# HyTruongSon/GraphFlow

Hardware: AMD Instinct MI355X
Metric: CCN-2D (SMP_omega) molecules/sec fwd+bwd (higher is better)
Workload: dtype f32 (level block products: 2xf16-split operands, 22-bit, fp32 accumulate); 1 GPU; cfg3: SMP_omega 3 levels, C=64, F=5, D=5, cap=29, batch=1024 synthetic QM9-size molecules/GPU, device-resident, fused levels; parallelism=single GPU

## Files before the change

### graphflow_amd/csrc/gf_internal.h

```cpp
#ifndef GF_INTERNAL_H_INCLUDED
#define GF_INTERNAL_H_INCLUDED

#include <hip/hip_runtime.h>

#include <cstdarg>
#include <cstddef>
#include <cstdio>
#include <cstdlib>
#include <unordered_map>
#include <vector>

#include "gf_hip.h"

struct gf_dist_state;

struct gf_ctx {
    int device = 0;
    gf_dist_state *dist = nullptr;
    int fp32_products = 0;
    int r18_generic = 0;
    hipStream_t stream = nullptr;
    bool owns_stream = false;
    void *ws = nullptr;
    size_t ws_bytes = 0;
    void *stage = nullptr;
    size_t stage_bytes = 0;
    void *repack = nullptr;
    size_t repack_bytes = 0;
    void *pinned = nullptr;
    size_t pinned_bytes = 0;
    char err[512] = {0};
    bool timing = false;
    char timing_filter[64] = {0};
    struct Timer {
        const char *name;
        double ms;
        long long launches;
    };
    struct Pending {
        int slot;
        hipEvent_t start, stop;
    };
    std::vector<Timer> timers;
    std::vector<Pending> pending;
    std::vector<hipEvent_t> event_pool;
};

namespace gf {

gf_status fail(gf_ctx *ctx, gf_status st, const char *fmt, ...);
inline bool env_is(const char *name, char v) {
    const char *e = std::getenv(name);
    return e && e[0] == v;
}
bool poison_buffers();
gf_status ensure_ws(gf_ctx *ctx, size_t bytes);
gf_status ensure_stage(gf_ctx *ctx, size_t bytes);
gf_status ensure_repack(gf_ctx *ctx, size_t bytes);
gf_status ensure_pinned(gf_ctx *ctx, size_t bytes);
gf_status opt_in_lds_fn(gf_ctx *ctx, const void *kernel, size_t bytes);
template <typename Kern>
gf_status opt_in_lds(gf_ctx *ctx, Kern kern, size_t bytes) {
    return opt_in_lds_fn(ctx, reinterpret_cast<const void *>(kern), bytes);
}
bool dist_active(const gf_ctx *ctx);
bool dist_poisoned(const gf_ctx *ctx);
gf_status dist_allreduce_on(gf_ctx *ctx, float *buf, size_t n, hipStream_t stream, const char *what = nullptr);
gf_status dist_wait_event(gf_ctx *ctx, hipEvent_t ev, const char *where);
hipStream_t dist_stream(gf_ctx *ctx);

#ifndef GF_NT_SITES
#define GF_NT_SITES 124
#endif
#if defined(__HIPCC__)
template <int SITE, typename V>
__device__ __forceinline__ V gf_ld_s(const V *p) {
    if constexpr ((GF_NT_SITES & SITE) != 0) return __builtin_nontemporal_load(p);
    else return *p;
}
template <int SITE, typename V>
__device__ __forceinline__ void gf_st_s(V *p, V v) {
    if constexpr ((GF_NT_SITES & SITE) != 0) __builtin_nontemporal_store(v, p);
    else *p = v;
}
#endif

#define GF_HIP_TRY(ctx, expr)                                                                      \
    do {                                                                                           \
        hipError_t e__ = (expr);                                                                   \
        if (e__ != hipSuccess)                                                                     \
            return gf::fail((ctx), GF_ERR_HIP, "%s failed: %s (%s:%d)", #expr, hipGetErrorString(e__), \
                            __FILE__, __LINE__);                                                   \
    } while (0)

#define GF_LAUNCH_CHECK(ctx, what)                                                                  \
    do {                                                                                            \
        hipError_t e__ = hipGetLastError();                                                         \
        if (e__ != hipSuccess)                                                                      \
            return gf::fail((ctx), GF_ERR_HIP, "launch of %s failed: %s", (what), hipGetErrorString(e__)); \
    } while (0)

struct LaunchTimer {
    gf_ctx *ctx;
    int slot = -1;
    hipEvent_t start = nullptr, stop = nullptr;
    hipStream_t stream = nullptr;
    LaunchTimer(gf_ctx *c, const char *name, hipStream_t on = nullptr);
    void done();
};
gf_status resolve_timers(gf_ctx *ctx);

#define GF_LAUNCH(ctx, name, kern, grid, block, lds, ...)                                  \
    do {                                                                                   \
        gf::LaunchTimer lt__((ctx), (name));                                               \
        hipLaunchKernelGGL(kern, grid, block, lds, (ctx)->stream, __VA_ARGS__);           \
        lt__.done();                                                                       \
        GF_LAUNCH_CHECK((ctx), (name));                                                    \
    } while (0)

static inline size_t align_up(size_t x, size_t a) { return (x + a - 1) / a * a; }

gf_status r18_forward(gf_ctx *ctx, const float *P, const float *A, float *Out, int N, int C, int batch);
gf_status r18_backward(gf_ctx *ctx, const float *G, const float *A, float *dP, int N, int C, int batch, int accumulate);
size_t r18_workspace_bytes(int N, int C, int batch);
struct gf_ragged_nodes {
    const int *pair_node;
    const int *node_s;
    const long long *node_p, *node_row, *node_pair;
    long long total_rows, total_pairs;
};
bool r18_ragged_supported(int smax, int C, const void *p0, const void *p1);
size_t r18_ragged_workspace_bytes(long long total_rows, long long total_pairs, int C);
gf_status r18_forward_ragged(gf_ctx *ctx, const float *P, const float *A, float *Out, const gf_ragged_nodes &t,
                             long long pair_lo, long long pair_hi, int smax, int C);
gf_status r18_backward_ragged(gf_ctx *ctx, const float *G, const float *A, float *dP, const gf_ragged_nodes &t,
                              long long pair_lo, long long pair_hi, int smax, int C, int accumulate);
gf_status family_forward(gf_ctx *ctx, int K, const float *P, const float *A, float *Out, int N, int C, int batch);
gf_status family_backward(gf_ctx *ctx, int K, const float *G, const float *A, float *dP, int N, int C, int batch,
                          int accumulate);
size_t family_workspace_bytes(int K, int N, int C, int batch);

}
#endif
```

### graphflow_amd/csrc/smp_level_c64_split.hip

```cpp
#include <cstdlib>
#include <type_traits>

#include "gemm_lds.h"
#include "gf_internal.h"
#include "smp_internal.h"

namespace gf {
namespace {

using lds_image::f16v;
using lds_image::f4v;
typedef _Float16 h8 __attribute__((ext_vector_type(8)));
typedef _Float16 h2 __attribute__((ext_vector_type(2)));
typedef float f2v __attribute__((ext_vector_type(2)));

constexpr int kSpThreads = 512;

template <unsigned EMIN = 14u>
__device__ __forceinline__ void pow2_scale(unsigned maxbits, float *s, float *inv) {
    unsigned e = maxbits >> 23;
    e = e < EMIN ? EMIN : e;
    *s = __uint_as_float((267u - e) << 23);
    *inv = __uint_as_float((e - 13u) << 23);
}
// ... 85 lines not shown
        else
            build_weight_images<false, 1, 16>(w, H, L, winv, wmax, threadIdx.x);
    } else {
        if (blockIdx.x == 0)
            build_weight_images<true, 1, 32>(w, H, L, winv, wmax, threadIdx.x);
        else
            build_weight_images<false, 1, 32>(w, H, L, winv, wmax, threadIdx.x);
    }
}

__global__ __launch_bounds__(kSpThreads) void smp_split_weight_images_c128(SplitImages a) {
    __shared__ unsigned wmax[1];
    const int q = blockIdx.z >> 3, pos = blockIdx.z & 7, i = q >> 1, j = q & 1;
    uint4 *out = a.img[blockIdx.y] + (size_t)(2 * q + blockIdx.x) * kSpImgStride128;
    float *winv = reinterpret_cast<float *>(out + 2 * kSpAll128) + pos;
    const float *w = a.Wst[blockIdx.y] + (size_t)pos * 128 * 128;
    uint4 *H = out + pos * 512, *L = out + kSpAll128 + pos * 512;
    if (blockIdx.x == 0)
        build_weight_images<true, 1, 64, 128>(w + (size_t)64 * i * 128 + 64 * j, H, L, winv, wmax, threadIdx.x);
    else
        build_weight_images<false, 1, 64, 128>(w + (size_t)64 * j * 128 + 64 * i, H, L, winv, wmax, threadIdx.x);
}

#ifndef GF_SP_WHOLE_PANEL
#define GF_SP_WHOLE_PANEL 16
#endif
template <bool FWD, bool MASK, int CB = 64, int NF = 2, int NX = 0, bool CLS = false, int W = 1, bool ACC = false>
__global__ __launch_bounds__(kSpThreads, 1) void smp_rowpanel_split(const float *__restrict__ A, const float *__restrict__ rs,
                                                                     const float *__restrict__ Wst, float *__restrict__ Out, int rows,
                                                                     const int *__restrict__ trow, int store_mask,
                                                                     const uint4 *__restrict__ wimg,
                                                                     const int *__restrict__ rcls,
                                                                     int a_off, int out_off) {
    static_assert(W == 1 || (CB == 64 && NF == 2 && NX == 0 && !CLS), "sub-block passes: 64-channel panels, plain row factors");
    static_assert(W > 1 || !ACC, "");
    static_assert(!CLS || (!FWD && MASK && CB == 64 && NF == 2 && NX == 0), "row classes: the masked backward products at 64 channels");
    constexpr int LDA = (FWD ? 4 * CB : 2 * CB) * W, LDOUT = (FWD ? 2 * CB : 4 * CB) * W, BS = CB * W;
    if constexpr (W == 1) a_off = out_off = 0;
    constexpr int ALL = W == 1 ? kSpAll : kSpAll128;
    constexpr int VPL = CB / 2, NC = CB / 16, NH = CB >= 32 ? CB / 32 : 1, E = NH * NC * 64;
    auto t_row = [](int t) { return MASK ? (t & 0x1fffffff) : t; };
    auto t_own = [](int t) { return MASK ? t < 0 : true; };
    auto t_tr = [](int t) { return MASK ? ((t >> 30) & 1) != 0 : true; };
    auto t_bc = [](int t) { return MASK ? ((t >> 29) & 1) != 0 : true; };
    static_assert(NX == 0 || (NX == 3 && CB <= 32 && NF == 2), "the extra products: prebuilt images, plain row factors");
    constexpr int NP = 8 + NX;
    extern __shared__ __attribute__((aligned(16))) uint4 sp_smem[];
    uint4 *imgH = sp_smem, *imgL = sp_smem + NP * E;
    float *winv = reinterpret_cast<float *>(sp_smem + 2 * NP * E);
    unsigned *wmax = reinterpret_cast<unsigned *>(winv + 16);
    float *facs = winv + 32;
    const int tid = threadIdx.x, lane = tid & 63, li = lane & 31, lh = lane >> 5;
    const int wave = tid >> 6;
    typedef unsigned long long u64x2 __attribute__((ext_vector_type(2)));
    unsigned long long *rowp = reinterpret_cast<unsigned long long *>(facs + (kSpThreads / 64) * 32);

    if (wimg) {
        for (int t = tid; t < NP * E; t += kSpThreads) {
            const int pos = t / E, g = (pos < 8 ? pos : kSpStacked + pos - 8) * 512 + t % E;
            imgH[t] = wimg[g];
            imgL[t] = wimg[ALL + g];
        }
        if (tid < 2) reinterpret_cast<uint4 *>(winv)[tid] = wimg[2 * ALL + tid];
        if (NX > 0 && tid < NX) winv[8 + tid] = reinterpret_cast<const float *>(wimg + 2 * kSpAll)[kSpStacked + tid];
    } else {
        static_assert(E == 512 || true, "");
        if constexpr (CB == 64) build_weight_images<FWD, 8>(Wst, imgH, imgL, winv, wmax, tid);
    }
    __syncthreads();

    const int npanels = (rows + 31) / 32;
    const int nwaves = gridDim.x * (kSpThreads / 64);
    float *myfac = facs + wave * 32;

    struct Raw {
        f4v a[VPL / 4];
    };
    struct Spl {
        uint4 h[NC], l[NC];
    };
    auto load_raw_at = [&](Raw &R, int src_row, int blk, bool present) {
        __builtin_amdgcn_sched_barrier(0);
        asm volatile("" : "+v"(src_row));
        const float *src = A + (size_t)src_row * LDA + blk * BS + a_off + VPL * lh;
        if constexpr (MASK) src = present ? src : sp_zero_page;
#pragma unroll
        for (int q = 0; q < VPL / 4; ++q) R.a[q] = gf_ld_s<1>(reinterpret_cast<const f4v *>(src + 4 * q));
        __builtin_amdgcn_sched_barrier(0);
    };
    auto load_raw = [&](Raw &R, int p, int blk, bool present) {
        const int row = p * 32 + li;
        load_raw_at(R, row < rows ? row : rows - 1, blk, present);
    };
    auto fetch_trow = [&](int p) {
        const int row = p * 32 + li;
        return trow[row < rows ? row : rows - 1];
    };
    struct RowFac {
        float f[8];
    };
    auto load_scale = [&](int p) {
        int row = p * 32 + li;
        row = row < rows ? row : rows - 1;
        RowFac r;
        if constexpr (NF == 8) {
            const f4v a = *reinterpret_cast<const f4v *>(rs + (size_t)row * 8), b = *reinterpret_cast<const f4v *>(rs + (size_t)row * 8 + 4);
            r.f[0] = a[0], r.f[1] = a[1], r.f[2] = a[2], r.f[3] = a[3], r.f[4] = b[0], r.f[5] = b[1], r.f[6] = b[2], r.f[7] = b[3];
        } else {
            const float2 t = *reinterpret_cast<const float2 *>(rs + (size_t)row * 2);
            r.f[0] = r.f[1] = t.x, r.f[2] = t.y;
            r.f[3] = r.f[4] = r.f[5] = r.f[6] = r.f[7] = 1.f;
        }
        return r;
    };
    auto split_blk = [&](const Raw &R, Spl &S, float &inv) {
        __builtin_amdgcn_sched_barrier(0);
        unsigned m = 0u;
#pragma unroll
        for (int q = 0; q < VPL / 4; ++q)
#pragma unroll
            for (int j = 0; j < 4; ++j) {
                const unsigned b = __float_as_uint(R.a[q][j]) & 0x7fffffffu;
                m = b > m ? b : m;
            }
        const unsigned mo = (unsigned)__shfl_xor((int)m, 32);
        m = mo > m ? mo : m;
        float s;
        pow2_scale(m, &s, &inv);
#pragma unroll
        for (int c = 0; c < NC; ++c) {
            unsigned hw[4], lw[4];
#pragma unroll
            for (int j = 0; j < 4; ++j) {
                h2 h, l;
                const f4v v = R.a[2 * c + (j >> 1)];
                split_pair(v[2 * (j & 1)], v[2 * (j & 1) + 1], s, &h, &l);
                hw[j] = __builtin_bit_cast(unsigned, h);
                lw[j] = __builtin_bit_cast(unsigned, l);
            }
            S.h[c] = make_uint4(hw[0], hw[1], hw[2], hw[3]);
            S.l[c] = make_uint4(lw[0], lw[1], lw[2], lw[3]);
        }
        __builtin_amdgcn_sched_barrier(0);
    };
    auto prod = [&](const Spl &S, float rowfac, int wpos, f16v &acc0, f16v &acc1) {
        __builtin_amdgcn_wave_barrier();
        myfac[li] = rowfac * winv[wpos];
        __builtin_amdgcn_wave_barrier();
        const uint4 *bh = imgH + (size_t)wpos * E + lane, *bl = imgL + (size_t)wpos * E + lane;
#pragma unroll
        for (int nh = 0; nh < NH; ++nh) {
            f16v t;
#pragma unroll
            for (int r = 0; r < 16; ++r) t[r] = 0.f;
#pragma unroll
            for (int c = 0; c < NC; ++c) {
                const h8 bhc = __builtin_bit_cast(h8, bh[(NC * nh + c) * 64]), blc = __builtin_bit_cast(h8, bl[(NC * nh + c) * 64]);
                const h8 ah = __builtin_bit_cast(h8, S.h[c]), al = __builtin_bit_cast(h8, S.l[c]);
                t = __builtin_amdgcn_mfma_f32_32x32x16_f16(al, bhc, t, 0, 0, 0);
                t = __builtin_amdgcn_mfma_f32_32x32x16_f16(ah, blc, t, 0, 0, 0);
            }
#pragma unroll
            for (int r = 0; r < 16; ++r) t[r] *= kLowUnscale;
#pragma unroll
            for (int c = 0; c < NC; ++c) {
                const h8 bhc = __builtin_bit_cast(h8, bh[(NC * nh + c) * 64]);
                const h8 ah = __builtin_bit_cast(h8, S.h[c]);
                t = __builtin_amdgcn_mfma_f32_32x32x16_f16(ah, bhc, t, 0, 0, 0);
            }
            f16v &acc = nh ? acc1 : acc0;
#pragma unroll
            for (int g = 0; g < 4; ++g) {
                const f4v fac = *reinterpret_cast<const f4v *>(myfac + 8 * g + 4 * lh);
#pragma unroll
                for (int j = 0; j < 4; ++j) acc[4 * g + j] += t[4 * g + j] * fac[j];
            }
        }
        __builtin_amdgcn_wave_barrier();
    };
    auto clear = [&](f16v &acc0, f16v &acc1) {
#pragma unroll
        for (int r = 0; r < 16; ++r) acc0[r] = acc1[r] = 0.f;
    };
    auto start = [&](int p, int o, f16v &acc0, f16v &acc1, auto full) {
        if constexpr (!ACC) {
            clear(acc0, acc1);
        } else {
            const int r0 = p * 32;
            const float *out = Out + (size_t)(r0 + 4 * lh) * LDOUT + o * BS + out_off + li;
#pragma unroll
            for (int r = 0; r < 16; ++r) {
                const int rr = (r & 3) + 8 * (r >> 2);
                const bool ok = decltype(full)::value || r0 + 4 * lh + rr < rows;
                acc0[r] = ok ? out[(size_t)rr * LDOUT] : 0.f;
                acc1[r] = ok ? out[(size_t)rr * LDOUT + 32] : 0.f;
            }
        }
    };
    auto store_out = [&](int p, int o, const f16v &acc0, const f16v &acc1, auto full, unsigned rowbits = 0xffffffffu) {
        const int r0 = p * 32;
        float *out = Out + (size_t)(r0 + 4 * lh) * LDOUT + o * BS + out_off + li;
        if constexpr (CB < 32)
            out = li < CB ? out : sp_dump + (size_t)((r0 & 255) + 4 * lh) * 64 + li;
        if constexpr (MASK && !FWD && decltype(full)::value) {
            if (rowbits != 0xffffffffu) {
                const unsigned mine = rowbits >> (4 * lh);
                float *dump = sp_dump + (size_t)((r0 & 255) + 4 * lh) * 64 + li;
#pragma unroll
                for (int r = 0; r < 16; ++r) {
                    const int rr = (r & 3) + 8 * (r >> 2);
                    float *dst = ((mine >> rr) & 1u) ? out + (size_t)rr * LDOUT : dump + rr * 64;
                    gf_st_s<2>(dst, acc0[r]);
                    if constexpr (NH == 2) gf_st_s<2>(dst + 32, acc1[r]);
                }
                return;
            }
        }
        if constexpr (decltype(full)::value) {
#pragma unroll
            for (int r = 0; r < 16; ++r) {
                const int rr = (r & 3) + 8 * (r >> 2);
                gf_st_s<2>(out + (size_t)rr * LDOUT, acc0[r]);
                if constexpr (NH == 2) gf_st_s<2>(out + (size_t)rr * LDOUT + 32, acc1[r]);
            }
        } else {
            const unsigned mine = (MASK && !FWD) ? rowbits >> (4 * lh) : 0xffffffffu;
#pragma unroll
            for (int r = 0; r < 16; ++r) {
                const int rr = (r & 3) + 8 * (r >> 2);
                if (r0 + 4 * lh + rr < rows && li < CB && ((mine >> rr) & 1u)) {
                    gf_st_s<2>(out + (size_t)rr * LDOUT, acc0[r]);
                    if constexpr (NH == 2) gf_st_s<2>(out + (size_t)rr * LDOUT + 32, acc1[r]);
                }
            }
        }
    };

    int tnext = CLS ? 0 : fetch_trow(blockIdx.x * (kSpThreads / 64) + wave);
    auto panel = [&](int p, Raw &Ra, Raw &Rb, auto full) {
        const int pn = p + nwaves;
        const int tcur = tnext;
        tnext = fetch_trow(pn);
        const RowFac sc = load_scale(p);
        f16v acc0, acc1;
        Spl X, Y, Z;
        float iX, iY, iZ;
        if (FWD) {
            split_blk(Ra, X, iX);
            load_raw(Ra, p, 1, t_bc(tcur));
            split_blk(Rb, Z, iZ);
            load_raw(Rb, p, 2, t_own(tcur));
            start(p, 1, acc0, acc1, full);
            prod(X, iX * sc.f[5], 5, acc0, acc1);
            prod(Z, iZ * sc.f[7], 7, acc0, acc1);
            split_blk(Ra, Y, iY);
            prod(Y, iY * sc.f[6], 6, acc0, acc1);
            store_out(p, 1, acc0, acc1, full);
            start(p, 0, acc0, acc1, full);
            prod(X, iX * sc.f[0], 0, acc0, acc1);
            prod(X, iX * sc.f[2], 2, acc0, acc1);
            prod(Y, iY * sc.f[1], 1, acc0, acc1);
            if constexpr (NX == 3) {
                prod(X, iX, 8, acc0, acc1);
                prod(Y, iY, 9, acc0, acc1);
                prod(Y, iY * sc.f[2], 10, acc0, acc1);
            }
            load_raw(Ra, p, 3, t_bc(tcur));
            split_blk(Rb, Z, iZ);
            load_raw_at(Rb, t_row(tnext), 0, t_tr(tnext));
            prod(Z, iZ * sc.f[3], 3, acc0, acc1);
            split_blk(Ra, Z, iZ);
            load_raw(Ra, pn, 0, t_own(tnext));
            prod(Z, iZ * sc.f[4], 4, acc0, acc1);
            store_out(p, 0, acc0, acc1, full);
        } else {
            split_blk(Ra, X, iX);
            split_blk(Rb, Y, iY);
            const unsigned rowbits = (MASK && store_mask) ? (unsigned)__ballot(t_own(tcur)) : 0xffffffffu;
            start(p, 2, acc0, acc1, full);
            prod(X, iX * sc.f[3], 3, acc0, acc1);
            store_out(p, 2, acc0, acc1, full, rowbits);
            start(p, 3, acc0, acc1, full);
            prod(X, iX * sc.f[4], 4, acc0, acc1);
            store_out(p, 3, acc0, acc1, full);
            start(p, 1, acc0, acc1, full);
            prod(X, iX * sc.f[1], 1, acc0, acc1);
            prod(Y, iY * sc.f[6], 6, acc0, acc1);
            if constexpr (NX == 3) {
                prod(X, iX, 9, acc0, acc1);
                prod(X, iX * sc.f[2], 10, acc0, acc1);
            }
            store_out(p, 1, acc0, acc1, full);
            load_raw_at(Ra, t_row(tcur), 1, !(MASK && store_mask) || t_own(tcur));
            load_raw(Rb, pn, 1, !(MASK && store_mask) || t_bc(tnext));
            start(p, 0, acc0, acc1, full);
            prod(X, iX * sc.f[0], 0, acc0, acc1);
            prod(X, iX * sc.f[2], 2, acc0, acc1);
            prod(Y, iY * sc.f[5], 5, acc0, acc1);
            if constexpr (NX == 3) prod(X, iX, 8, acc0, acc1);
            split_blk(Ra, Z, iZ);
            load_raw(Ra, pn, 0, !(MASK && store_mask) || t_bc(tnext));
            prod(Z, iZ * sc.f[7], 7, acc0, acc1);
            store_out(p, 0, acc0, acc1, full, rowbits);
        }
    };
    if constexpr (CLS) {
        const int n_own_p = (rcls[0] + 31) >> 5, n_tot_p = n_own_p + ((rcls[1] + 31) >> 5), n_ent = 32 * n_tot_p;
        const int2 *ent = reinterpret_cast<const int2 *>(rcls + 4);
        unsigned long long *myrow = rowp + wave * 32;
        auto fetch_entry = [&](int q, int *rw) {
            const int i = q * 32 + li;
            const int2 e = ent[i < n_ent ? i : n_ent - 1];
            *rw = e.x;
            return e.y;
        };
        auto e_row = [](int rw) { return rw & 0x1fffffff; };
        auto scale_at = [&](int row) {
            const float2 t = *reinterpret_cast<const float2 *>(rs + (size_t)row * 2);
            RowFac r;
            r.f[0] = r.f[1] = t.x, r.f[2] = t.y;
            r.f[3] = r.f[4] = r.f[5] = r.f[6] = r.f[7] = 1.f;
            return r;
        };
        auto post_rows = [&](int rw) {
            __builtin_amdgcn_wave_barrier();
            myrow[li] = reinterpret_cast<unsigned long long>(rw < 0 ? sp_dump + li * 64 : Out + (size_t)e_row(rw) * LDOUT);
            __builtin_amdgcn_wave_barrier();
        };
        auto store_rows = [&](int o, const f16v &acc0, const f16v &acc1) {
#pragma unroll
            for (int g = 0; g < 4; ++g) {
                const u64x2 a = *reinterpret_cast<const u64x2 *>(myrow + 8 * g + 4 * lh), b = *reinterpret_cast<const u64x2 *>(myrow + 8 * g + 4 * lh + 2);
#pragma unroll
                for (int j = 0; j < 4; ++j) {
                    float *dst = reinterpret_cast<float *>(j < 2 ? a[j & 1] : b[j & 1]) + o * CB + li;
                    gf_st_s<2>(dst, acc0[4 * g + j]);
                    gf_st_s<2>(dst + 32, acc1[4 * g + j]);
                }
            }
        };
        int p = blockIdx.x * (kSpThreads / 64) + wave;
        int rnext, tn = fetch_entry(p, &rnext);
        Raw Ra, Rb;
        load_raw_at(Rb, e_row(rnext), 1, t_bc(tn));
        load_raw_at(Ra, e_row(rnext), 0, t_bc(tn));
        auto panel_own = [&](int q) {
            const int qn = q + nwaves, rcur = rnext, tcur = tn;
            tn = fetch_entry(qn, &rnext);
            const RowFac sc = scale_at(e_row(rcur));
            post_rows(rcur);
            f16v acc0, acc1;
            Spl X, Y, Z;
            float iX, iY, iZ;
            split_blk(Ra, X, iX);
            split_blk(Rb, Y, iY);
            clear(acc0, acc1);
            prod(X, iX * sc.f[3], 3, acc0, acc1);
            store_rows(2, acc0, acc1);
            clear(acc0, acc1);
            prod(X, iX * sc.f[4], 4, acc0, acc1);
            store_rows(3, acc0, acc1);
            clear(acc0, acc1);
            prod(X, iX * sc.f[1], 1, acc0, acc1);
            prod(Y, iY * sc.f[6], 6, acc0, acc1);
            store_rows(1, acc0, acc1);
            load_raw_at(Ra, t_row(tcur), 1, t_own(tcur));
            load_raw_at(Rb, e_row(rnext), 1, t_bc(tn));
            clear(acc0, acc1);
            prod(X, iX * sc.f[0], 0, acc0, acc1);
            prod(X, iX * sc.f[2], 2, acc0, acc1);
            prod(Y, iY * sc.f[5], 5, acc0, acc1);
            split_blk(Ra, Z, iZ);
            load_raw_at(Ra, e_row(rnext), 0, t_bc(tn));
            prod(Z, iZ * sc.f[7], 7, acc0, acc1);
            store_rows(0, acc0, acc1);
        };
        auto panel_absent = [&](int q) {
            const int qn = q + nwaves, rcur = rnext;
            tn = fetch_entry(qn, &rnext);
            const RowFac sc = scale_at(e_row(rcur));
            post_rows(rcur);
            f16v acc0, acc1;
            Spl X, Y;
            float iX, iY;
            split_blk(Ra, X, iX);
            split_blk(Rb, Y, iY);
            load_raw_at(Rb, e_row(rnext), 1, t_bc(tn));
            load_raw_at(Ra, e_row(rnext), 0, t_bc(tn));
            clear(acc0, acc1);
            prod(X, iX * sc.f[4], 4, acc0, acc1);
            store_rows(3, acc0, acc1);
            clear(acc0, acc1);
            prod(X, iX * sc.f[1], 1, acc0, acc1);
            prod(Y, iY * sc.f[6], 6, acc0, acc1);
            store_rows(1, acc0, acc1);
        };
        for (; p < n_own_p; p += nwaves) panel_own(p);
        for (; p < n_tot_p; p += nwaves) panel_absent(p);
        return;
    }
    if constexpr (CB <= GF_SP_WHOLE_PANEL) {
        constexpr int NB = FWD ? 5 : 3;
        Raw R[NB];
        int p = blockIdx.x * (kSpThreads / 64) + wave;
        int t1 = tnext, t2 = fetch_trow(p + nwaves);
        auto request = [&](int q, int t) {
            if constexpr (FWD) {
                load_raw(R[0], q, 0, t_own(t));
                load_raw_at(R[1], t_row(t), 0, t_tr(t));
                load_raw(R[2], q, 1, t_bc(t));
                load_raw(R[3], q, 2, t_own(t));
                load_raw(R[4], q, 3, t_bc(t));
            } else {
                const bool all = !(MASK && store_mask);
                load_raw(R[0], q, 0, all || t_bc(t));
                load_raw(R[1], q, 1, all || t_bc(t));
                load_raw_at(R[2], t_row(t), 1, all || t_own(t));
            }
        };
        auto panel16 = [&](int q, auto full) {
// ... 154 lines not shown
                const h8 ah = __builtin_bit_cast(h8, S.h[c]);
                t = __builtin_amdgcn_mfma_f32_32x32x16_f16(ah, bhc, t, 0, 0, 0);
            }
            f16v &acc = nh ? acc1 : acc0;
#pragma unroll
            for (int g = 0; g < 4; ++g) {
                const f4v fac = *reinterpret_cast<const f4v *>(myfac + 8 * g + 4 * lh);
#pragma unroll
                for (int j = 0; j < 4; ++j) acc[4 * g + j] += t[4 * g + j] * fac[j];
            }
        }
        __builtin_amdgcn_wave_barrier();
    };
    const int npanels = (rows + 31) / 32;
    for (int p = wg * (kSmThreads / 64) + wave; p < npanels; p += nwg * (kSmThreads / 64)) {
        const int r0 = p * 32;
        const int row = r0 + li < rows ? r0 + li : rows - 1;
        Raw R[NIN];
#pragma unroll
        for (int k = 0; k < NIN; ++k) {
            const float *src = In + (size_t)row * LDA + k * CB + VPL * lh;
#pragma unroll
            for (int q = 0; q < VPL / 4; ++q) R[k].a[q] = *reinterpret_cast<const f4v *>(src + 4 * q);
        }
        (void)NIN;
        auto store_out = [&](int o, const f16v &acc0, const f16v &acc1) {
            float *out = Out + (size_t)(r0 + 4 * lh) * LDOUT + o * CB + li;
#pragma unroll
            for (int r = 0; r < 16; ++r) {
                const int rr = (r & 3) + 8 * (r >> 2);
                if (r0 + 4 * lh + rr < rows && li < CB) {
                    out[(size_t)rr * LDOUT] = acc0[r];
                    if constexpr (NH == 2) out[(size_t)rr * LDOUT + 32] = acc1[r];
                }
            }
        };
        f16v acc0, acc1;
        Spl X;
        float iX;
        if constexpr (PROG == 0) {
#pragma unroll
            for (int r = 0; r < 16; ++r) acc0[r] = acc1[r] = 0.f;
#pragma unroll
            for (int k = 0; k < NPOS; ++k) {
                split_blk(R[k], X, iX);
                prod(X, iX, k, acc0, acc1);
            }
            store_out(0, acc0, acc1);
        } else if constexpr (PROG == 1) {
            split_blk(R[0], X, iX);
#pragma unroll
            for (int k = 0; k < NPOS; ++k) {
#pragma unroll
                for (int r = 0; r < 16; ++r) acc0[r] = acc1[r] = 0.f;
                prod(X, iX, k, acc0, acc1);
                store_out(k, acc0, acc1);
            }
        } else {
#pragma unroll
            for (int k = 0; k < NPOS; ++k) {
                split_blk(R[k], X, iX);
#pragma unroll
                for (int r = 0; r < 16; ++r) acc0[r] = acc1[r] = 0.f;
                prod(X, iX, k, acc0, acc1);
                store_out(k, acc0, acc1);
            }
        }
    }
}

template <int CB>
__global__ __launch_bounds__(kSmThreads, 2) void smp_small_split(SmallJobs jobs, const uint4 *__restrict__ wimg) {
    int j = 0;
    if (jobs.n > 1 && (int)blockIdx.x >= jobs.wg0[1]) j = 1;
    if (jobs.n > 2 && (int)blockIdx.x >= jobs.wg0[2]) j = 2;
    const int wg = (int)blockIdx.x - jobs.wg0[j];
    switch (jobs.prog[j]) {
        case 0: small_split_body<0, CB>(jobs.In[j], jobs.Out[j], jobs.rows[j], wimg, jobs.pos0[j], wg, jobs.nwg[j]); break;
        case 1: small_split_body<1, CB>(jobs.In[j], jobs.Out[j], jobs.rows[j], wimg, jobs.pos0[j], wg, jobs.nwg[j]); break;
        default: small_split_body<2, CB>(jobs.In[j], jobs.Out[j], jobs.rows[j], wimg, jobs.pos0[j], wg, jobs.nwg[j]); break;
    }
}

constexpr int kWsThreads = 512, kWsSlice = 16, kWsRowWords = 12;
constexpr int kWsACols = 256, kWsBCols = 320;
constexpr int kWsStageWords = 2 * (kWsACols + kWsBCols) * kWsRowWords;
constexpr size_t kWsLds = 2 * (size_t)kWsStageWords * 4 + 2 * (kWsACols + kWsBCols) * sizeof(float);
__constant__ int c_ws_ablk[8] = {0, 1, 0, 2, 3, 0, 1, 0};
__constant__ int c_ws_bblk[8] = {1, 1, 2, 0, 0, 3, 3, 4};

template <int W = 1>
__global__ __launch_bounds__(kWsThreads, 1) void smp_wgrad_split(const float *__restrict__ T, const float *__restrict__ dO,
                                                                  const float *__restrict__ rs, int rows, int kchunk,
                                                                  float *__restrict__ part, const int *__restrict__ trow,
                                                                  const unsigned *__restrict__ cmax,
                                                                  const unsigned *__restrict__ chan,
                                                                  float smax, float max_tot, float max_tr,
                                                                  const unsigned *__restrict__ row_max,
                                                                  int packed,
                                                                  int a_off, int b_off, int out_off) {
    if constexpr (W == 1) a_off = b_off = out_off = 0;
    constexpr int LDT = 256 * W, LDO = 128 * W, BS = 64 * W, LDW = 64 * W;
    extern __shared__ __attribute__((aligned(16))) unsigned ws_smem[];
    const int tid = threadIdx.x, lane = tid & 63, li = lane & 31, lg = lane >> 5;
    const int wave = __builtin_amdgcn_readfirstlane(tid >> 6);
    const int kend = rows;
    auto K = [&](int n) { return (long long)(blockIdx.x + (long long)n * gridDim.x) * kWsSlice; };

    float *sScale = reinterpret_cast<float *>(ws_smem + 2 * kWsStageWords), *sInv = sScale + kWsACols + kWsBCols;
    if (cmax) {
        for (int c = tid; c < kWsACols + kWsBCols; c += kWsThreads) pow2_scale_col(cmax[c], &sScale[c], &sInv[c]);
    } else {
        if (row_max) {
            max_tot = __uint_as_float(row_max[0]);
            max_tr = __uint_as_float(row_max[1]);
        }
        for (int c = tid; c < kWsACols + kWsBCols; c += kWsThreads) {
            const bool isa = c < kWsACols;
            const int blk = (isa ? c : c - kWsACols) >> 6, ch = c & 63;
            const float m = __uint_as_float(chan[(isa ? 0 : 64) + ch]);
            const float fa = blk < 2 ? smax : max_tot;
            const float fb = blk == 0 ? 1.f : blk == 2 ? max_tr : max_tot;
            pow2_scale_col(__float_as_uint(m * (isa ? fa : fb)), &sScale[c], &sInv[c]);
        }
    }
    __syncthreads();

    const int q_lo = lane & 7, pair = lane >> 3;
    struct Task {
        f4v v0, v1;
    };
    constexpr int NB = 2;
    struct Set {
        Task ta, tb[NB];
        float f0[NB], f1[NB];
    };
    const bool has_b1 = wave < 2;
    const int zbit = ((wave >> 1) & 1) == 0 ? 31 : 29;
    const int a_quad = 8 * wave + q_lo;
    auto b_blk = [&](int e) { return (wave + 8 * e) >> 1; };
    auto b_quad = [&](int e) { return 8 * ((wave + 8 * e) & 1) + q_lo; };
    const int rot = (q_lo >> 1) & 3;
    f4v a_scale, b_scale[NB];
#pragma unroll
    for (int i = 0; i < 4; ++i) {
        a_scale[i] = sScale[4 * a_quad + ((i + rot) & 3)];
#pragma unroll
        for (int e = 0; e < NB; ++e) {
            const int blk = b_blk(e) < 5 ? b_blk(e) : 0;
            b_scale[e][i] = sScale[kWsACols + 64 * blk + 4 * b_quad(e) + ((i + rot) & 3)];
        }
    }
    int ia0 = 0, ia1 = 0, ib0 = 0, ib1 = 0;
    auto fetch_trow = [&](int m, int &t0, int &t1) {
        const long long k = K(m) + 2 * pair, last = kend - 1;
        t0 = trow[k < last ? k : last];
        t1 = trow[k + 1 < last ? k + 1 : last];
    };
    auto load_slice = [&](Set &S, int m) {
        const int g0 = packed ? (ia0 & 0x1fffffff) : ia0, g1 = packed ? (ia1 & 0x1fffffff) : ia1;
        const bool z0 = packed && !((ia0 >> zbit) & 1), z1 = packed && !((ia1 >> zbit) & 1);
        const bool zg0 = packed && ia0 >= 0, zg1 = packed && ia1 >= 0;
        ia0 = ib0, ia1 = ib1;
        fetch_trow(m + 2, ib0, ib1);
        const long long last = kend - 1, kk = K(m) + 2 * pair;
        const int c0 = (int)(kk < last ? kk : last), c1 = (int)(kk + 1 < last ? kk + 1 : last);
        const int a_col = W == 1 ? 4 * a_quad : (a_quad >> 4) * BS + a_off + ((4 * a_quad) & 63);
        const float *t0 = T + (size_t)c0 * LDT + a_col, *t1 = T + (size_t)c1 * LDT + a_col;
        S.ta.v0 = gf_ld_s<4>(reinterpret_cast<const f4v *>(z0 ? sp_zero_page + 4 * q_lo : t0));
        S.ta.v1 = gf_ld_s<4>(reinterpret_cast<const f4v *>(z1 ? sp_zero_page + 4 * q_lo : t1));
#pragma unroll
        for (int e = 0; e < NB; ++e) {
            const int blk = b_blk(e);
            S.f0[e] = rs[(size_t)c0 * 2 + (blk == 2)];
            S.f1[e] = rs[(size_t)c1 * 2 + (blk == 2)];
            const bool gathered = blk == 4;
            const float *src = blk < 5 ? dO + (blk >= 3 ? BS : 0) + b_off + 4 * b_quad(e) : T + a_col;
            const int ld = blk < 5 ? LDO : LDT;
            const float *s0 = src + (size_t)(gathered ? g0 : c0) * ld, *s1 = src + (size_t)(gathered ? g1 : c1) * ld;
            S.tb[e].v0 = gf_ld_s<256>(reinterpret_cast<const f4v *>((gathered && zg0) ? sp_zero_page + 4 * q_lo : s0));
            S.tb[e].v1 = gf_ld_s<256>(reinterpret_cast<const f4v *>((gathered && zg1) ? sp_zero_page + 4 * q_lo : s1));
        }
    };
    auto rotate = [&](f4v v) {
        if (rot & 1) v = f4v{v[1], v[2], v[3], v[0]};
        if (rot & 2) v = f4v{v[2], v[3], v[0], v[1]};
        return v;
    };
    auto store_task = [&](const f4v &v0, const f4v &v1, unsigned *H, unsigned *L, int col0, const f4v &sc, float f0, float f1) {
        const f4v r0 = rotate(v0), r1 = rotate(v1);
#pragma unroll
        for (int i = 0; i < 4; ++i) {
            h2 h, l;
            split_plain2(r0[i], r1[i], sc[i] * f0, sc[i] * f1, &h, &l);
            const int w = (col0 + ((i + rot) & 3)) * kWsRowWords + pair;
            H[w] = __builtin_bit_cast(unsigned, h);
            L[w] = __builtin_bit_cast(unsigned, l);
        }
    };
    auto store_slice = [&](const Set &S, long long k0, unsigned *stage) {
        unsigned *Ah = stage, *Al = Ah + kWsACols * kWsRowWords, *Bh = Al + kWsACols * kWsRowWords, *Bl = Bh + kWsBCols * kWsRowWords;
        const long long k = k0 + 2 * pair;
        const float ok0 = k < kend ? 1.f : 0.f, ok1 = k + 1 < kend ? 1.f : 0.f;
        store_task(S.ta.v0, S.ta.v1, Ah, Al, 4 * a_quad, a_scale, ok0, ok1);
#pragma unroll
        for (int e = 0; e < NB; ++e) {
            if (e == 1 && !has_b1) break;
            const int blk = b_blk(e);
            const bool scaled = blk == 1 || blk == 2;
            const float m0 = scaled ? S.f0[e] : 1.f, m1 = scaled ? S.f1[e] : 1.f;
            store_task(S.tb[e].v0, S.tb[e].v1, Bh, Bl, 64 * blk + 4 * b_quad(e), b_scale[e], ok0 * m0, ok1 * m1);
        }
    };

    f16v acc[2][2];
#pragma unroll
    for (int r = 0; r < 16; ++r) acc[0][0][r] = acc[0][1][r] = acc[1][0][r] = acc[1][1][r] = 0.f;
    const int ablk = c_ws_ablk[wave], bblk = c_ws_bblk[wave];
    auto products = [&](const unsigned *stage) {
        const unsigned *Ah = stage, *Al = Ah + kWsACols * kWsRowWords, *Bh = Al + kWsACols * kWsRowWords, *Bl = Bh + kWsBCols * kWsRowWords;
        const int ao = (ablk * 64 + li) * kWsRowWords + 4 * lg, bo = (bblk * 64 + li) * kWsRowWords + 4 * lg;
        h8 ah[2], al[2], bh[2], bl[2];
#pragma unroll
        for (int t = 0; t < 2; ++t) {
            ah[t] = __builtin_bit_cast(h8, *reinterpret_cast<const uint4 *>(Ah + ao + t * 32 * kWsRowWords));
            al[t] = __builtin_bit_cast(h8, *reinterpret_cast<const uint4 *>(Al + ao + t * 32 * kWsRowWords));
            bh[t] = __builtin_bit_cast(h8, *reinterpret_cast<const uint4 *>(Bh + bo + t * 32 * kWsRowWords));
            bl[t] = __builtin_bit_cast(h8, *reinterpret_cast<const uint4 *>(Bl + bo + t * 32 * kWsRowWords));
        }
#pragma unroll
        for (int mt = 0; mt < 2; ++mt)
#pragma unroll
            for (int nt = 0; nt < 2; ++nt) {
                acc[mt][nt] = __builtin_amdgcn_mfma_f32_32x32x16_f16(al[mt], bh[nt], acc[mt][nt], 0, 0, 0);
                acc[mt][nt] = __builtin_amdgcn_mfma_f32_32x32x16_f16(ah[mt], bl[nt], acc[mt][nt], 0, 0, 0);
                acc[mt][nt] = __builtin_amdgcn_mfma_f32_32x32x16_f16(ah[mt], bh[nt], acc[mt][nt], 0, 0, 0);
            }
    };
    auto interval = [&](Set &Ra, int n) {
        store_slice(Ra, K(n + 1), ws_smem + ((n + 1) & 1) * kWsStageWords);
        load_slice(Ra, n + 4);
        products(ws_smem + (n & 1) * kWsStageWords);
        __syncthreads();
    };
    if (K(0) < kend) {
        Set S0, S1, S2;
        fetch_trow(0, ia0, ia1);
        fetch_trow(1, ib0, ib1);
        load_slice(S0, 0);
        load_slice(S1, 1);
        load_slice(S2, 2);
        store_slice(S0, K(0), ws_smem);
        load_slice(S0, 3);
        __syncthreads();
        int left = (int)((kend - K(0) + (long long)gridDim.x * kWsSlice - 1) / ((long long)gridDim.x * kWsSlice));
        int n = 0;
        for (; left >= 3; n += 3, left -= 3) {
            interval(S1, n);
            interval(S2, n + 1);
            interval(S0, n + 2);
        }
        if (left >= 1) interval(S1, n);
        if (left >= 2) interval(S2, n + 1);
    }
    float *out = part + ((size_t)blockIdx.x * 8 + wave) * (LDW * LDW) + out_off + li;
    const float *ia = sInv + ablk * 64, *ib = sInv + kWsACols + bblk * 64;
#pragma unroll
    for (int mt = 0; mt < 2; ++mt)
#pragma unroll
        for (int nt = 0; nt < 2; ++nt) {
            const float ub = ib[32 * nt + li];
#pragma unroll
            for (int r = 0; r < 16; ++r) {
                const int row = 32 * mt + (r & 3) + 8 * (r >> 2) + 4 * lg;
                out[row * LDW + 32 * nt] = acc[mt][nt][r] * (ia[row] * ub);
            }
        }
}


constexpr long long kTrowWindow = (long long)kFusedMaxField * kFusedMaxField;
constexpr int kW8Threads = 256;
template <int CB, int NF, int NX = 0>
__global__ __launch_bounds__(kW8Threads, 1) void smp_wgrad_all(const float *__restrict__ T, const float *__restrict__ dO,
                                                                const float *__restrict__ rs, int rows, float *__restrict__ part,
                                                                const int *__restrict__ trow, const unsigned *__restrict__ cmax,
                                                                const unsigned *__restrict__ chan, float smax,
                                                                const unsigned *__restrict__ row_max, int packed, float *__restrict__ xpart = nullptr) {
    static_assert(CB == 32 || CB == 16, "one 32 x 32 tile per product");
    static_assert(NX == 0 || (NX == 3 && NF == 2), "the extra products take the plain (tot, tr) row factors");
    constexpr int NP = 8 + NX;
    constexpr int ACOLS = 4 * CB, BCOLS = 5 * CB;
    constexpr int SL = CB == 16 ? 2 * kWsSlice : kWsSlice;
    constexpr int TROW = 16 * CB, DROW = 8 * CB;
    constexpr int NBF = NF == 8 ? 8 : 5;
    __shared__ float sScale[ACOLS + BCOLS], sInv[ACOLS + BCOLS];
    __shared__ float sImg[NP * CB * CB];
    const int tid = threadIdx.x, lane = tid & 63, li = lane & 31, lg = lane >> 5;
    const int wave = __builtin_amdgcn_readfirstlane(tid >> 6);
    const int hi = (CB == 16 && li >= 16) ? 1 : 0;
    const int lc = CB == 16 ? (li & 15) : li;
    const int rb = 8 * lg + 16 * hi;
    if (cmax) {
        for (int c = tid; c < ACOLS + BCOLS; c += kW8Threads) pow2_scale_col(cmax[c], &sScale[c], &sInv[c]);
    } else {
        const float max_tot = __uint_as_float(row_max[0]), max_tr = __uint_as_float(row_max[1]);
        for (int c = tid; c < ACOLS + BCOLS; c += kW8Threads) {
            const bool isa = c < ACOLS;
            const int blk = (isa ? c : c - ACOLS) / CB, ch = c % CB;
            const float m = __uint_as_float(chan[(isa ? 0 : CB) + ch]);
            const float fa = blk < 2 ? smax : max_tot;
// ... 577 lines not shown
```

Baseline: 155,700 molecules/s.

## Swizzle weight-gradient LDS staging layout and tag global pointers with address space

```diff
diff --git a/graphflow_amd/csrc/gf_internal.h b/graphflow_amd/csrc/gf_internal.h
--- a/graphflow_amd/csrc/gf_internal.h
+++ b/graphflow_amd/csrc/gf_internal.h
@@ -83,6 +83,25 @@
     if constexpr ((GF_NT_SITES & SITE) != 0) __builtin_nontemporal_store(v, p);
     else *p = v;
 }
+#define GF_GLOBAL __attribute__((address_space(1)))
+template <typename V>
+__device__ __forceinline__ const GF_GLOBAL V *gf_global(const V *p) {
+    return (const GF_GLOBAL V *)p;
+}
+template <typename V>
+__device__ __forceinline__ GF_GLOBAL V *gf_global(V *p) {
+    return (GF_GLOBAL V *)p;
+}
+template <int SITE, typename V>
+__device__ __forceinline__ V gf_ld_g(const GF_GLOBAL V *p) {
+    if constexpr ((GF_NT_SITES & SITE) != 0) return __builtin_nontemporal_load(p);
+    else return *p;
+}
+template <int SITE, typename V>
+__device__ __forceinline__ void gf_st_g(GF_GLOBAL V *p, V v) {
+    if constexpr ((GF_NT_SITES & SITE) != 0) __builtin_nontemporal_store(v, p);
+    else *p = v;
+}
 #endif
 
 #define GF_HIP_TRY(ctx, expr)                                                                      \
diff --git a/graphflow_amd/csrc/smp_level_c64_split.hip b/graphflow_amd/csrc/smp_level_c64_split.hip
--- a/graphflow_amd/csrc/smp_level_c64_split.hip
+++ b/graphflow_amd/csrc/smp_level_c64_split.hip
@@ -191,10 +191,11 @@
     auto load_raw_at = [&](Raw &R, int src_row, int blk, bool present) {
         __builtin_amdgcn_sched_barrier(0);
         asm volatile("" : "+v"(src_row));
-        const float *src = A + (size_t)src_row * LDA + blk * BS + a_off + VPL * lh;
-        if constexpr (MASK) src = present ? src : sp_zero_page;
-#pragma unroll
-        for (int q = 0; q < VPL / 4; ++q) R.a[q] = gf_ld_s<1>(reinterpret_cast<const f4v *>(src + 4 * q));
+        unsigned long long sa = (unsigned long long)(A + (size_t)src_row * LDA + blk * BS + a_off + VPL * lh);
+        if constexpr (MASK) sa = present ? sa : (unsigned long long)sp_zero_page;
+        const GF_GLOBAL float *src = (const GF_GLOBAL float *)sa;
+#pragma unroll
+        for (int q = 0; q < VPL / 4; ++q) R.a[q] = gf_ld_g<1>(reinterpret_cast<const GF_GLOBAL f4v *>(src + 4 * q));
         __builtin_amdgcn_sched_barrier(0);
     };
     auto load_raw = [&](Raw &R, int p, int blk, bool present) {
@@ -282,7 +283,10 @@
             for (int g = 0; g < 4; ++g) {
                 const f4v fac = *reinterpret_cast<const f4v *>(myfac + 8 * g + 4 * lh);
 #pragma unroll
-                for (int j = 0; j < 4; ++j) acc[4 * g + j] += t[4 * g + j] * fac[j];
+                for (int j = 0; j < 4; ++j) {
+                    if constexpr (!FWD && CB == 16) acc[4 * g + j] = __builtin_fmaf(t[4 * g + j], fac[j], acc[4 * g + j]);
+                    else acc[4 * g + j] += t[4 * g + j] * fac[j];
+                }
             }
         }
         __builtin_amdgcn_wave_barrier();
@@ -308,19 +312,19 @@
     };
     auto store_out = [&](int p, int o, const f16v &acc0, const f16v &acc1, auto full, unsigned rowbits = 0xffffffffu) {
         const int r0 = p * 32;
-        float *out = Out + (size_t)(r0 + 4 * lh) * LDOUT + o * BS + out_off + li;
+        GF_GLOBAL float *out = gf_global(Out) + (size_t)(r0 + 4 * lh) * LDOUT + o * BS + out_off + li;
         if constexpr (CB < 32)
-            out = li < CB ? out : sp_dump + (size_t)((r0 & 255) + 4 * lh) * 64 + li;
+            out = li < CB ? out : gf_global(sp_dump) + (size_t)((r0 & 255) + 4 * lh) * 64 + li;
         if constexpr (MASK && !FWD && decltype(full)::value) {
             if (rowbits != 0xffffffffu) {
                 const unsigned mine = rowbits >> (4 * lh);
-                float *dump = sp_dump + (size_t)((r0 & 255) + 4 * lh) * 64 + li;
+                GF_GLOBAL float *dump = gf_global(sp_dump) + (size_t)((r0 & 255) + 4 * lh) * 64 + li;
 #pragma unroll
                 for (int r = 0; r < 16; ++r) {
                     const int rr = (r & 3) + 8 * (r >> 2);
-                    float *dst = ((mine >> rr) & 1u) ? out + (size_t)rr * LDOUT : dump + rr * 64;
-                    gf_st_s<2>(dst, acc0[r]);
-                    if constexpr (NH == 2) gf_st_s<2>(dst + 32, acc1[r]);
+                    GF_GLOBAL float *dst = ((mine >> rr) & 1u) ? out + (size_t)rr * LDOUT : dump + rr * 64;
+                    gf_st_g<2>(dst, acc0[r]);
+                    if constexpr (NH == 2) gf_st_g<2>(dst + 32, acc1[r]);
                 }
                 return;
             }
@@ -329,8 +333,8 @@
 #pragma unroll
             for (int r = 0; r < 16; ++r) {
                 const int rr = (r & 3) + 8 * (r >> 2);
-                gf_st_s<2>(out + (size_t)rr * LDOUT, acc0[r]);
-                if constexpr (NH == 2) gf_st_s<2>(out + (size_t)rr * LDOUT + 32, acc1[r]);
+                gf_st_g<2>(out + (size_t)rr * LDOUT, acc0[r]);
+                if constexpr (NH == 2) gf_st_g<2>(out + (size_t)rr * LDOUT + 32, acc1[r]);
             }
         } else {
             const unsigned mine = (MASK && !FWD) ? rowbits >> (4 * lh) : 0xffffffffu;
@@ -338,8 +342,8 @@
             for (int r = 0; r < 16; ++r) {
                 const int rr = (r & 3) + 8 * (r >> 2);
                 if (r0 + 4 * lh + rr < rows && li < CB && ((mine >> rr) & 1u)) {
-                    gf_st_s<2>(out + (size_t)rr * LDOUT, acc0[r]);
-                    if constexpr (NH == 2) gf_st_s<2>(out + (size_t)rr * LDOUT + 32, acc1[r]);
+                    gf_st_g<2>(out + (size_t)rr * LDOUT, acc0[r]);
+                    if constexpr (NH == 2) gf_st_g<2>(out + (size_t)rr * LDOUT + 32, acc1[r]);
                 }
             }
         }
@@ -433,7 +437,7 @@
         };
         auto post_rows = [&](int rw) {
             __builtin_amdgcn_wave_barrier();
-            myrow[li] = reinterpret_cast<unsigned long long>(rw < 0 ? sp_dump + li * 64 : Out + (size_t)e_row(rw) * LDOUT);
+            myrow[li] = (unsigned long long)(rw < 0 ? gf_global(sp_dump) + li * 64 : gf_global(Out) + (size_t)e_row(rw) * LDOUT);
             __builtin_amdgcn_wave_barrier();
         };
         auto store_rows = [&](int o, const f16v &acc0, const f16v &acc1) {
@@ -442,9 +446,9 @@
                 const u64x2 a = *reinterpret_cast<const u64x2 *>(myrow + 8 * g + 4 * lh), b = *reinterpret_cast<const u64x2 *>(myrow + 8 * g + 4 * lh + 2);
 #pragma unroll
                 for (int j = 0; j < 4; ++j) {
-                    float *dst = reinterpret_cast<float *>(j < 2 ? a[j & 1] : b[j & 1]) + o * CB + li;
-                    gf_st_s<2>(dst, acc0[4 * g + j]);
-                    gf_st_s<2>(dst + 32, acc1[4 * g + j]);
+                    GF_GLOBAL float *dst = (GF_GLOBAL float *)(j < 2 ? a[j & 1] : b[j & 1]) + o * CB + li;
+                    gf_st_g<2>(dst, acc0[4 * g + j]);
+                    gf_st_g<2>(dst + 32, acc1[4 * g + j]);
                 }
             }
         };
@@ -765,9 +769,16 @@
     }
 }
 
-constexpr int kWsThreads = 512, kWsSlice = 16, kWsRowWords = 12;
+constexpr int kWsThreads = 512, kWsSlice = 16;
 constexpr int kWsACols = 256, kWsBCols = 320;
-constexpr int kWsStageWords = 2 * (kWsACols + kWsBCols) * kWsRowWords;
+constexpr unsigned long long kWsQuadSlot = 0x3713022611352400ull;
+constexpr int kWsBlockWords = 288;
+__device__ __forceinline__ int ws_col_word(int col) {
+    const int q = (col >> 2) & 7;
+    return (col >> 5) * kWsBlockWords + 4 * (int)((kWsQuadSlot >> (8 * q)) & 0xffu) + 16 * (col & 3);
+}
+constexpr int kWsAWords = kWsACols / 32 * kWsBlockWords, kWsBWords = kWsBCols / 32 * kWsBlockWords;
+constexpr int kWsStageWords = 2 * (kWsAWords + kWsBWords);
 constexpr size_t kWsLds = 2 * (size_t)kWsStageWords * 4 + 2 * (kWsACols + kWsBCols) * sizeof(float);
 __constant__ int c_ws_ablk[8] = {0, 1, 0, 2, 3, 0, 1, 0};
 __constant__ int c_ws_bblk[8] = {1, 1, 2, 0, 0, 3, 3, 4};
@@ -823,15 +834,14 @@
     const int a_quad = 8 * wave + q_lo;
     auto b_blk = [&](int e) { return (wave + 8 * e) >> 1; };
     auto b_quad = [&](int e) { return 8 * ((wave + 8 * e) & 1) + q_lo; };
-    const int rot = (q_lo >> 1) & 3;
     f4v a_scale, b_scale[NB];
 #pragma unroll
     for (int i = 0; i < 4; ++i) {
-        a_scale[i] = sScale[4 * a_quad + ((i + rot) & 3)];
+        a_scale[i] = sScale[4 * a_quad + i];
 #pragma unroll
         for (int e = 0; e < NB; ++e) {
             const int blk = b_blk(e) < 5 ? b_blk(e) : 0;
-            b_scale[e][i] = sScale[kWsACols + 64 * blk + 4 * b_quad(e) + ((i + rot) & 3)];
+            b_scale[e][i] = sScale[kWsACols + 64 * blk + 4 * b_quad(e) + i];
         }
     }
     int ia0 = 0, ia1 = 0, ib0 = 0, ib1 = 0;
@@ -849,40 +859,35 @@
         const long long last = kend - 1, kk = K(m) + 2 * pair;
         const int c0 = (int)(kk < last ? kk : last), c1 = (int)(kk + 1 < last ? kk + 1 : last);
         const int a_col = W == 1 ? 4 * a_quad : (a_quad >> 4) * BS + a_off + ((4 * a_quad) & 63);
-        const float *t0 = T + (size_t)c0 * LDT + a_col, *t1 = T + (size_t)c1 * LDT + a_col;
-        S.ta.v0 = gf_ld_s<4>(reinterpret_cast<const f4v *>(z0 ? sp_zero_page + 4 * q_lo : t0));
-        S.ta.v1 = gf_ld_s<4>(reinterpret_cast<const f4v *>(z1 ? sp_zero_page + 4 * q_lo : t1));
+        const GF_GLOBAL float *zero = gf_global(sp_zero_page) + 4 * q_lo;
+        const GF_GLOBAL float *t0 = gf_global(T) + (size_t)c0 * LDT + a_col, *t1 = gf_global(T) + (size_t)c1 * LDT + a_col;
+        S.ta.v0 = gf_ld_g<4>(reinterpret_cast<const GF_GLOBAL f4v *>(z0 ? zero : t0));
+        S.ta.v1 = gf_ld_g<4>(reinterpret_cast<const GF_GLOBAL f4v *>(z1 ? zero : t1));
 #pragma unroll
         for (int e = 0; e < NB; ++e) {
             const int blk = b_blk(e);
             S.f0[e] = rs[(size_t)c0 * 2 + (blk == 2)];
             S.f1[e] = rs[(size_t)c1 * 2 + (blk == 2)];
             const bool gathered = blk == 4;
-            const float *src = blk < 5 ? dO + (blk >= 3 ? BS : 0) + b_off + 4 * b_quad(e) : T + a_col;
+            const GF_GLOBAL float *src = blk < 5 ? gf_global(dO) + (blk >= 3 ? BS : 0) + b_off + 4 * b_quad(e) : gf_global(T) + a_col;
             const int ld = blk < 5 ? LDO : LDT;
-            const float *s0 = src + (size_t)(gathered ? g0 : c0) * ld, *s1 = src + (size_t)(gathered ? g1 : c1) * ld;
-            S.tb[e].v0 = gf_ld_s<256>(reinterpret_cast<const f4v *>((gathered && zg0) ? sp_zero_page + 4 * q_lo : s0));
-            S.tb[e].v1 = gf_ld_s<256>(reinterpret_cast<const f4v *>((gathered && zg1) ? sp_zero_page + 4 * q_lo : s1));
-        }
-    };
-    auto rotate = [&](f4v v) {
-        if (rot & 1) v = f4v{v[1], v[2], v[3], v[0]};
-        if (rot & 2) v = f4v{v[2], v[3], v[0], v[1]};
-        return v;
+            const GF_GLOBAL float *s0 = src + (size_t)(gathered ? g0 : c0) * ld, *s1 = src + (size_t)(gathered ? g1 : c1) * ld;
+            S.tb[e].v0 = gf_ld_g<256>(reinterpret_cast<const GF_GLOBAL f4v *>((gathered && zg0) ? zero : s0));
+            S.tb[e].v1 = gf_ld_g<256>(reinterpret_cast<const GF_GLOBAL f4v *>((gathered && zg1) ? zero : s1));
+        }
     };
     auto store_task = [&](const f4v &v0, const f4v &v1, unsigned *H, unsigned *L, int col0, const f4v &sc, float f0, float f1) {
-        const f4v r0 = rotate(v0), r1 = rotate(v1);
+        const int w = ws_col_word(col0) + pair;
 #pragma unroll
         for (int i = 0; i < 4; ++i) {
             h2 h, l;
-            split_plain2(r0[i], r1[i], sc[i] * f0, sc[i] * f1, &h, &l);
-            const int w = (col0 + ((i + rot) & 3)) * kWsRowWords + pair;
-            H[w] = __builtin_bit_cast(unsigned, h);
-            L[w] = __builtin_bit_cast(unsigned, l);
+            split_plain2(v0[i], v1[i], sc[i] * f0, sc[i] * f1, &h, &l);
+            H[w + 16 * i] = __builtin_bit_cast(unsigned, h);
+            L[w + 16 * i] = __builtin_bit_cast(unsigned, l);
         }
     };
     auto store_slice = [&](const Set &S, long long k0, unsigned *stage) {
-        unsigned *Ah = stage, *Al = Ah + kWsACols * kWsRowWords, *Bh = Al + kWsACols * kWsRowWords, *Bl = Bh + kWsBCols * kWsRowWords;
+        unsigned *Ah = stage, *Al = Ah + kWsAWords, *Bh = Al + kWsAWords, *Bl = Bh + kWsBWords;
         const long long k = k0 + 2 * pair;
         const float ok0 = k < kend ? 1.f : 0.f, ok1 = k + 1 < kend ? 1.f : 0.f;
         store_task(S.ta.v0, S.ta.v1, Ah, Al, 4 * a_quad, a_scale, ok0, ok1);
@@ -901,15 +906,15 @@
     for (int r = 0; r < 16; ++r) acc[0][0][r] = acc[0][1][r] = acc[1][0][r] = acc[1][1][r] = 0.f;
     const int ablk = c_ws_ablk[wave], bblk = c_ws_bblk[wave];
     auto products = [&](const unsigned *stage) {
-        const unsigned *Ah = stage, *Al = Ah + kWsACols * kWsRowWords, *Bh = Al + kWsACols * kWsRowWords, *Bl = Bh + kWsBCols * kWsRowWords;
-        const int ao = (ablk * 64 + li) * kWsRowWords + 4 * lg, bo = (bblk * 64 + li) * kWsRowWords + 4 * lg;
+        const unsigned *Ah = stage, *Al = Ah + kWsAWords, *Bh = Al + kWsAWords, *Bl = Bh + kWsBWords;
+        const int ao = ws_col_word(ablk * 64 + li) + 4 * lg, bo = ws_col_word(bblk * 64 + li) + 4 * lg;
         h8 ah[2], al[2], bh[2], bl[2];
 #pragma unroll
         for (int t = 0; t < 2; ++t) {
-            ah[t] = __builtin_bit_cast(h8, *reinterpret_cast<const uint4 *>(Ah + ao + t * 32 * kWsRowWords));
-            al[t] = __builtin_bit_cast(h8, *reinterpret_cast<const uint4 *>(Al + ao + t * 32 * kWsRowWords));
-            bh[t] = __builtin_bit_cast(h8, *reinterpret_cast<const uint4 *>(Bh + bo + t * 32 * kWsRowWords));
-            bl[t] = __builtin_bit_cast(h8, *reinterpret_cast<const uint4 *>(Bl + bo + t * 32 * kWsRowWords));
+            ah[t] = __builtin_bit_cast(h8, *reinterpret_cast<const uint4 *>(Ah + ao + t * kWsBlockWords));
+            al[t] = __builtin_bit_cast(h8, *reinterpret_cast<const uint4 *>(Al + ao + t * kWsBlockWords));
+            bh[t] = __builtin_bit_cast(h8, *reinterpret_cast<const uint4 *>(Bh + bo + t * kWsBlockWords));
+            bl[t] = __builtin_bit_cast(h8, *reinterpret_cast<const uint4 *>(Bl + bo + t * kWsBlockWords));
         }
 #pragma unroll
         for (int mt = 0; mt < 2; ++mt)
```

Measured after the change: 157,600 molecules/s (median of 6 runs). 1.2% higher.
